# microsoft/gated-graph-neural-network-samples

Measured on AMD Instinct MI355X. Metric: node-state updates/sec on QM9-shaped graphs, h=100, 4 edge types, higher is better.
Workload: dtype f32

## Files before the change

gated-graph-neural-network-samples_amd/csrc/ggnn_gru_fused.hip:

```cpp
#include "ggnn_split.hpp"
#include "ggnn_gru_cells.hpp"
#include <type_traits>

#ifndef GGNN_COOP_DEPTH
#define GGNN_COOP_DEPTH 1
#endif
#ifndef GGNN_GRU_STAMPS
#define GGNN_GRU_STAMPS 0
#endif
#if GGNN_GRU_STAMPS
#define GGNN_TDBG(a) (a).tdbg
#else
#define GGNN_TDBG(a) ((unsigned long long*)nullptr)
#endif

#ifndef GGNN_GRU_ABLATE
#define GGNN_GRU_ABLATE 0
#endif
#if GGNN_GRU_ABLATE
#define GGNN_ABL(BIT) ((ablate & (BIT)) != 0)
#define GGNN_ABL_PARAM , int ablate
#define GGNN_ABL_ARG , gru_ablate_bits()
static int gru_ablate_bits() { static const int v = [] { const char* e = getenv("GGNN_GRU_DBG"); return e ? atoi(e) : 0; }(); return v; }
#else
// ... 19 lines not shown
                  ImgCfg<32, true>::IMG >= ImgCfg<32, true, kSplitF16x2>::IMG, "bf16x3 images are the larger ones");
    switch (D) {
        case 100: return 3 * (nx + 1) * (sp ? ImgCfg<100, true>::IMG : ImgCfg<100, false>::IMG);
        case 64: return 3 * (nx + 1) * (sp ? ImgCfg<64, true>::IMG : ImgCfg<64, false>::IMG);
        case 32: return 3 * (nx + 1) * (sp ? ImgCfg<32, true>::IMG : ImgCfg<32, false>::IMG);
        default: return 0;
    }
}
#endif

template <int D, bool SPLIT, int FMT = kSplitBf16x3>
__global__ void gru_pack_weights_kernel(const float* __restrict__ Wg, const float* __restrict__ Wc, int nx,
                                        float* __restrict__ out) {
    const int ci = blockIdx.y;
    float* img = out + (size_t)ci * ImgCfg<D, SPLIT, FMT>::IMG;
    if constexpr (SPLIT) gru_fwd_image_pack_split<D, FMT>(Wg, Wc, nx, ci, img, blockIdx.x * blockDim.x + threadIdx.x, gridDim.x * blockDim.x);
    else gru_fwd_image_pack<D>(Wg, Wc, nx, ci, img, blockIdx.x * blockDim.x + threadIdx.x, gridDim.x * blockDim.x);
}

template <int NX>
__host__ __device__ constexpr int gru_stage_image(int pos) {
    return (pos % 3) < 2 ? 2 * (pos / 3) + (pos % 3) : 2 * (NX + 1) + pos / 3;
}

template <int FMT>
__device__ __forceinline__ f32x4 sigmoid4_acc(f32x4 z, f32x4 b_scaled) {
    constexpr float k = -kLog2e * SplitFmt<FMT>::acc_scale;
    return rcp_4(exp2_4(z * k + b_scaled) + 1.0f);
}
template <int FMT>
__device__ __forceinline__ f32x4 tanh4_acc(f32x4 z, f32x4 b_scaled) {
    constexpr float k = 2.0f * kLog2e * SplitFmt<FMT>::acc_scale;
    return 1.0f - 2.0f * rcp_4(exp2_4(z * k + b_scaled) + 1.0f);
}

template <int D>
__device__ __forceinline__ void frag_zero(Frag<D>& f) {
#pragma unroll
    for (int c = 0; c < StageCfg<D>::NC; ++c) f.v[c] = f32x4{0.f, 0.f, 0.f, 0.f};
#pragma unroll
    for (int q = 0; q < StageCfg<D>::NR; ++q) f.r[q] = 0.f;
}

template <int D>
__device__ __forceinline__ void frag_add(Frag<D>& f, const Frag<D>& t) {
#pragma unroll
    for (int c = 0; c < StageCfg<D>::NC; ++c) f.v[c] += t.v[c];
#pragma unroll
    for (int q = 0; q < StageCfg<D>::NR; ++q) f.r[q] += t.r[q];
}

template <int D, int NX, int NW, bool SAVE, bool GATHER, bool SPLIT, bool SAVEX = SAVE, int FORM = 0, int FMT = kSplitBf16x3,
          int TK = kTkRuntime, bool G4AVG = false>
__global__ __launch_bounds__(NW * 64, FORM == 1 ? 2 : 1) void ggnn_gru_fused_kernel(GruFusedArgs a, const float* __restrict__ packed GGNN_ABL_PARAM) {
    static_assert(SPLIT || FMT == kSplitBf16x3, "the f32-MFMA kernels have no operand format");
    using C = StageCfg<D>;
    using I = ImgCfg<D, SPLIT, FMT>;
    using SC = SplitCfg<D, FMT>;
    constexpr bool HALF = FORM != 0;
    constexpr bool DEEP = FORM == 2;
    constexpr int NSLOT = DEEP ? 3 : 2;
    static_assert(!HALF || SPLIT, "the half-stage forms are split-form kernels");
    static_assert(FORM != 1 || NW == 4, "form 1 is the four-wave kernel");
    static_assert(!G4AVG || GATHER, "G4AVG fixes the gather's parameters");
    auto dyn_tk = [&]() -> bool {
        if constexpr (TK == kTkRuntime) return a.tickets != nullptr;
// ... 52 lines not shown
    };
    auto publish = [&]() { if constexpr (SPLIT) dma_wait(); __syncthreads(); };
    auto dma_ha = [&](const float* src, float* dst) { dma_kib_asm<SC::HA_BYTES / 1024, NW>(src, dst, wave, lane); };
    auto dma_hb = [&](const float* src, float* dst) { dma_kib_asm<SC::HB_BYTES / 1024, NW>(src, dst, wave, lane); };
    constexpr int KA = SC::HA_BYTES / 1024, KB = SC::HB_BYTES / 1024;
    const int own_a = KA / NW + (wave < KA % NW ? 1 : 0), own_b = KB / NW + (wave < KB % NW ? 1 : 0);
    auto publish_deep = [&](int own) {
        switch (own) {
            case 0: asm volatile("s_waitcnt vmcnt(0) lgkmcnt(0)" ::: "memory"); break;
            case 1: asm volatile("s_waitcnt vmcnt(1) lgkmcnt(0)" ::: "memory"); break;
            case 2: asm volatile("s_waitcnt vmcnt(2) lgkmcnt(0)" ::: "memory"); break;
            case 3: asm volatile("s_waitcnt vmcnt(3) lgkmcnt(0)" ::: "memory"); break;
            case 4: asm volatile("s_waitcnt vmcnt(4) lgkmcnt(0)" ::: "memory"); break;
            case 5: asm volatile("s_waitcnt vmcnt(5) lgkmcnt(0)" ::: "memory"); break;
            case 6: asm volatile("s_waitcnt vmcnt(6) lgkmcnt(0)" ::: "memory"); break;
            case 7: asm volatile("s_waitcnt vmcnt(7) lgkmcnt(0)" ::: "memory"); break;
            case 8: asm volatile("s_waitcnt vmcnt(8) lgkmcnt(0)" ::: "memory"); break;
            case 9: asm volatile("s_waitcnt vmcnt(9) lgkmcnt(0)" ::: "memory"); break;
            default: asm volatile("s_waitcnt vmcnt(10) lgkmcnt(0)" ::: "memory"); break;
        }
        __builtin_amdgcn_s_barrier();
    };
    static_assert(!DEEP || (SC::HA_BYTES / 1024 + NW - 1) / NW <= 10, "publish_deep covers <= 10 pieces per wave");
    if constexpr (DEEP) {
        dma_ha(packed, ring);
        dma_hb(packed + SC::HA, ring + SLOT);
    } else if constexpr (HALF) dma_ha(packed, ring);
    else dma(packed, ring);

    constexpr int GSEG = NX - 1, GBUF = GSEG & 1;
    constexpr int KI = 4;
    constexpr int G_U = NX == 1 ? NSTAGE : 3 * (NX - 1);
    constexpr bool G_NEXT = (NX == 1);
    int g_beg = 0, g_end = 0;
    int g_i[KI] = {0, 0, 0, 0};
    f32x4 g_n = {0.f, 0.f, 0.f, 0.f};
    float g_den = 1.f, g_rcp = 1.f;
    Frag<D> gt;

    auto g_ptrs = [&](int r, bool on) {
        const int b = ldi_b(a.g_row_ptr, (unsigned)r * 4u), e = ldi_b(a.g_row_ptr, (unsigned)r * 4u + 4u);
        g_beg = on ? b : 0; g_end = on ? e : 0;
        if constexpr (G4AVG) {
            g_n = ld4_b(a.g_nin, (unsigned)r * 16u);
        } else if (a.g_use_avg) {
            if (a.g_T == 4) {
                g_n = ld4_b(a.g_nin, (unsigned)r * 16u);
            } else {
                float deg = 0.f;
                for (int t = 0; t < a.g_T; ++t) deg += a.g_nin[(size_t)r * a.g_T + t];
                g_n = f32x4{deg, 0.f, 0.f, 0.f};
            }
        }
    };
    auto touch = [](auto v) { asm volatile("" :: "v"(v)); };
    auto g_index = [&](int part) {
        if (part != 2) {
            touch(g_beg); touch(g_end);
            g_den = (((g_n.x + g_n.y) + g_n.z) + g_n.w) + 1e-7f;
            if constexpr (NX == 1) g_rcp = 1.0f / g_den;
        }
        if (part != 1) {
#pragma unroll
            for (int j = 0; j < KI; ++j) {
                g_i[j] = 0;
                if (g_beg + j < g_end) g_i[j] = ldi_b(a.g_idx, (unsigned)(g_beg + j) * 4u);
            }
        }
    };
    auto g_rows0 = [&](Frag<D>& f, int part) {
        if (part != 2) { touch(g_i[0]); touch(g_i[1]); touch(g_i[2]); touch(g_i[3]); }
        if (part != 1) {
            load_frag<D>(f, a.g_H, g_i[0], kq);
            load_frag<D>(gt, a.g_H, g_i[1], kq);
        }
    };
    auto g_rows = [&](Frag<D>& f, int k, int part) {
        if (part != 2) { if (g_beg + k - 1 < g_end) frag_add<D>(f, gt); }
        if (part != 1) load_frag<D>(gt, a.g_H, g_i[k], kq);
    };
    auto g_finish = [&](Frag<D>& f) {
        if (g_beg + KI - 1 < g_end) frag_add<D>(f, gt);
        for (int e = g_beg + KI; e < g_end; ++e) {
            load_frag<D>(gt, a.g_H, a.g_idx[e], kq);
            frag_add<D>(f, gt);
        }
        if (g_beg >= g_end) frag_zero<D>(f);
        if (G4AVG || a.g_use_avg) {
            const float den = g_den, r = g_rcp;
            auto dv = [&](float x) {
                if constexpr (NX == 1) { const float q = x * r; return fmaf(fmaf(-den, q, x), r, q); }
                else return x / den;
            };
#pragma unroll
            for (int c = 0; c < NC; ++c) f.v[c] = f32x4{dv(f.v[c].x), dv(f.v[c].y), dv(f.v[c].z), dv(f.v[c].w)};
#pragma unroll
            for (int q = 0; q < NR; ++q) f.r[q] = dv(f.r[q]);
        }
    };

    auto store_x = [&](const Frag<D>& f, int row_) {
        const unsigned ob = ((unsigned)row_ * (unsigned)D + 4u * (unsigned)kq) * 4u;
#pragma unroll
        for (int c = 0; c < NC; ++c) st4_b(a.save_x, ob + 64u * c, f.v[c]);
#pragma unroll
        for (int q = 0; q < NR; ++q) *reinterpret_cast<float*>(reinterpret_cast<char*>(a.save_x) + ob - 16u * (unsigned)kq + (16u * NC + 4u * q + (unsigned)kq) * 4u) = f.r[q];
    };
    Frag<D> hf, xf[2];
    {
        const int t0 = tile_of(tk);
        const bool on = t0 >= 0;
        const int r0 = (on ? t0 : 0) * 16 + li;
        const int r0c = r0 < a.V ? r0 : a.V - 1;
        if constexpr (GATHER) {
            if constexpr (G_NEXT) {
                g_ptrs(r0c, on);
                if (on) { g_index(0); g_rows0(xf[0], 0); g_rows(xf[0], 2, 0); g_rows(xf[0], 3, 0); g_finish(xf[0]); }
                if constexpr (SAVEX) { if (on && r0 < a.V && a.save_x) store_x(xf[0], r0); }
            } else {
                if constexpr (G_U - 5 < 0) g_ptrs(r0c, on);
                if constexpr (G_U - 4 < 0) g_index(0);
                load_frag<D>(xf[0], a.x[0], r0c, kq);
            }
        } else {
// ... 220 lines not shown
        GGNN_STAGE(0, acc_r, xf[0]) GGNN_STAGE(1, acc_u, xf[0]) GGNN_STAGE(2, acc_c, xf[0])
        if constexpr (NX >= 2) { GGNN_STAGE(3, acc_r, xf[1]) GGNN_STAGE(4, acc_u, xf[1]) GGNN_STAGE(5, acc_c, xf[1]) }
        if constexpr (NX >= 3) { GGNN_STAGE(6, acc_r, xf[0]) GGNN_STAGE(7, acc_u, xf[0]) GGNN_STAGE(8, acc_c, xf[0]) }
        GGNN_STAGE(3 * NX, acc_r, hf)
        GGNN_STAGE(3 * NX + 1, acc_u, hf)

        Frag<D> rh;
        if constexpr (coop) {
            const int col = wave * 16 + 4 * kq;
            if (wave < NT && col < D && !GGNN_ABL(2)) {
                const f32x4 r = sigmoid4_acc<FMT>(acc_r[0], ld4(bias_s + col));
                const f32x4 u = sigmoid4_acc<FMT>(acc_u[0], ld4(bias_s + D + col));
                f32x4 hv;
                if constexpr (COOP_REGS) hv = hv_pre;
                else hv = ld4_b(a.h, ((unsigned)rowc * D + col) * 4u);
                if constexpr (SAVE) {
                    if (row < a.V && a.save_r) {
                        st4_b(a.save_r, ((unsigned)row * D + col) * 4u, r);
                        st4_b(a.save_u, ((unsigned)row * D + col) * 4u, u);
                    }
                }
                acc_u[0] = u; acc_r[0] = hv;
                *reinterpret_cast<f32x4*>(rh_x + li * RHP + col) = r * hv;
            }
            __syncthreads();
#pragma unroll
            for (int c = 0; c < NC; ++c) rh.v[c] = *reinterpret_cast<const f32x4*>(rh_x + li * RHP + 16 * c + 4 * kq);
#pragma unroll
            for (int q = 0; q < NR; ++q) rh.r[q] = rh_x[li * RHP + 16 * NC + 4 * q + kq];
        } else if (active && !GGNN_ABL(2)) {
            stage_tail_reduce<D>(acc_r);
            stage_tail_reduce<D>(acc_u);
            if constexpr (C::TAILPACK) {
                constexpr int SH = 16 * ((D % 16) / 4);
                f32x4 ut;
                ut.x = __shfl(acc_r[NT - 1].x, lane + SH); ut.y = __shfl(acc_r[NT - 1].y, lane + SH);
                ut.z = __shfl(acc_r[NT - 1].z, lane + SH); ut.w = __shfl(acc_r[NT - 1].w, lane + SH);
                acc_u[NT - 1] = ut;
            }
#pragma unroll
            for (int nt = 0; nt < NT; ++nt) {
                const int col = nt * 16 + 4 * kq;
                if (col < D) {
                    const f32x4 r = sigmoid4_acc<FMT>(acc_r[nt], ld4(bias_s + col));
                    const f32x4 u = sigmoid4_acc<FMT>(acc_u[nt], ld4(bias_s + D + col));
                    acc_r[nt] = r; acc_u[nt] = u;
                    if constexpr (!SAVE && SPLIT && GATHER) { touch(u.x); touch(u.y); touch(u.z); touch(u.w); }
                    if constexpr (SAVE) {
                        if (row < a.V && a.save_r) {
                            st4_b(a.save_r, ((unsigned)row * D + col) * 4u, r);
                            st4_b(a.save_u, ((unsigned)row * D + col) * 4u, u);
                        }
                    }
                }
            }
#pragma unroll
            for (int c = 0; c < NC; ++c) rh.v[c] = acc_r[c] * hf.v[c];
#pragma unroll
            for (int q = 0; q < NR; ++q) {
                const float t0 = __shfl(acc_r[NT - 1].x, li + 16 * q), t1 = __shfl(acc_r[NT - 1].y, li + 16 * q);
                const float t2 = __shfl(acc_r[NT - 1].z, li + 16 * q), t3 = __shfl(acc_r[NT - 1].w, li + 16 * q);
                const float rr = kq == 0 ? t0 : (kq == 1 ? t1 : (kq == 2 ? t2 : t3));
                rh.r[q] = rr * hf.r[q];
            }
        }

        if (dyn_tk() && tid == 0) tk_slot[(p + 1) & 1] = nb + tk_fetch;
        GGNN_STAGE(3 * NX + 2, acc_c, rh)
#undef GGNN_STAGE
#undef GGNN_HALF_STAGE
#undef GGNN_COOP_STAGE
        tk = tk_next;
        tk_next = dyn_tk() ? __builtin_amdgcn_readfirstlane(tk_slot[(p + 1) & 1]) : tk_next + nb;

        if constexpr (coop) {
            const int col = wave * 16 + 4 * kq;
            if (wave < NT && col < D && row < a.V && !GGNN_ABL(4)) {
                f32x4 c;
                if (a.act == GGNN_ACT_TANH) {
                    c = tanh4_acc<FMT>(acc_c[0], ld4(bias_s + 2 * D + col));
                } else {
                    c = acc_c[0] * SplitFmt<FMT>::acc_scale + ld4(bias_s + 3 * D + col);
                    c.x = fmaxf(c.x, 0.f); c.y = fmaxf(c.y, 0.f); c.z = fmaxf(c.z, 0.f); c.w = fmaxf(c.w, 0.f);
                }
                const f32x4 u = acc_u[0], hv = acc_r[0];
                st4_b(a.h_out, ((unsigned)row * D + col) * 4u, u * hv + (1.0f - u) * c);
                if constexpr (SAVE) { if (a.save_c) st4_b(a.save_c, ((unsigned)row * D + col) * 4u, c); }
            }
            return;
        }
        f32x4 hrem = {0.f, 0.f, 0.f, 0.f};
        if (active) {
            stage_tail_reduce<D>(acc_c);
            if constexpr (C::TAILPACK3) {
                constexpr int SH2 = 32 * ((D % 16) / 4);
                f32x4 ct;
                ct.x = __shfl(acc_r[NT - 1].x, lane + SH2); ct.y = __shfl(acc_r[NT - 1].y, lane + SH2);
                ct.z = __shfl(acc_r[NT - 1].z, lane + SH2); ct.w = __shfl(acc_r[NT - 1].w, lane + SH2);
                acc_c[NT - 1] = ct + acc_c[NT - 1];
            }
#pragma unroll
            for (int q = 0; q < NR; ++q) {
                const float h0 = __shfl(hf.r[q], li), h1 = __shfl(hf.r[q], li + 16);
                const float h2 = __shfl(hf.r[q], li + 32), h3 = __shfl(hf.r[q], li + 48);
                if (kq == q) hrem = f32x4{h0, h1, h2, h3};
            }
        }
        if (active && row < a.V && !GGNN_ABL(4)) {
#pragma unroll
            for (int nt = 0; nt < NT; ++nt) {
                const int col = nt * 16 + 4 * kq;
                if (col < D) {
                    f32x4 hv;
                    if (nt < NC) hv = hf.v[nt];
                    else hv = hrem;
                    f32x4 c;
                    if (a.act == GGNN_ACT_TANH) {
                        c = tanh4_acc<FMT>(acc_c[nt], ld4(bias_s + 2 * D + col));
                    } else {
                        c = acc_c[nt] * SplitFmt<FMT>::acc_scale + ld4(bias_s + 3 * D + col);
                        c.x = fmaxf(c.x, 0.f); c.y = fmaxf(c.y, 0.f); c.z = fmaxf(c.z, 0.f); c.w = fmaxf(c.w, 0.f);
                    }
                    const f32x4 u = acc_u[nt];
                    st4_b(a.h_out, ((unsigned)row * D + col) * 4u, u * hv + (1.0f - u) * c);
                    if constexpr (SAVE) { if (a.save_c) st4_b(a.save_c, ((unsigned)row * D + col) * 4u, c); }
                }
            }
        }
    };
    int p = 0;
    for (; tk < n_main; ++p) run_pass(std::false_type{}, p);
    if constexpr (!HALF) { for (; tk < n_tk; ++p) run_pass(std::true_type{}, p); }
    if (GGNN_TDBG(a) && tid == 0) {
        a.tdbg[4096 + blockIdx.x * 4 + 2] = __builtin_amdgcn_s_memtime();
        a.tdbg[4096 + blockIdx.x * 4 + 3] = __builtin_amdgcn_s_memrealtime();
    }
}

// ... 235 lines not shown
```

gated-graph-neural-network-samples_amd/csrc/ggnn_msg_compact.hip:

```cpp
#include "ggnn_split.hpp"
#include <cstring>
#include <rocprim/device/device_scan.hpp>

namespace ggnn {

#ifndef GGNN_K1C_STAMPS
#define GGNN_K1C_STAMPS 0
#endif

constexpr int kMaxTypesC = 64;
struct TypeRows {
    int row_off[kMaxTypesC + 1]; int tile_off[kMaxTypesC + 1]; int T; int num_nodes;
#if GGNN_K1C_STAMPS
    unsigned long long* tdbg;
#endif
};

static inline size_t align256c(size_t x) { return (x + 255) / 256 * 256; }

__global__ void compact_flags_kernel(const int* __restrict__ src_row_ptr, int V, int T, int* flags) {
    const long long p = (long long)blockIdx.x * blockDim.x + threadIdx.x;
    if (p >= (long long)V * T) return;
    const int t = (int)(p / V), v = (int)(p - (long long)t * V);
    const int s = v * T + t;
    flags[p] = src_row_ptr[s + 1] > src_row_ptr[s] ? 1 : 0;
}

__global__ void compact_fill_kernel(const int* __restrict__ flags, const int* __restrict__ scan, int V, int T,
                                    int* pair_node, int* pair_id, int* type_row_off) {
    const long long p = (long long)blockIdx.x * blockDim.x + threadIdx.x;
    const long long n = (long long)V * T;
    if (p >= n) return;
    const int t = (int)(p / V), v = (int)(p - (long long)t * V);
    const int f = flags[p], c = scan[p];
    pair_id[v * T + t] = f ? c : -1;
    if (f) pair_node[c] = v;
    if (v == 0) type_row_off[t] = c;
    if (p == n - 1) type_row_off[T] = c + f;
}

__global__ void remap_rows_kernel(const int* __restrict__ gather_row, const int* __restrict__ pair_id, int* out, long long M) {
    const long long i = (long long)blockIdx.x * blockDim.x + threadIdx.x;
    if (i < M) out[i] = pair_id[gather_row[i]];
}

static size_t scan_temp_bytes(long long n) {
    size_t bytes = 0;
    (void)rocprim::exclusive_scan(nullptr, bytes, (const int*)nullptr, (int*)nullptr, 0, (size_t)n, rocprim::plus<int>(), (hipStream_t)0);
    return bytes;
}

template <int D, bool SPLIT, int FMT = kSplitBf16x3>
__global__ void edge_weight_pack_kernel(const float* __restrict__ W, float* __restrict__ out) {
    const int t = blockIdx.y;
    float* img = out + (size_t)t * ImgCfg<D, SPLIT, FMT>::IMG;
    const int first = blockIdx.x * blockDim.x + threadIdx.x, stride = gridDim.x * blockDim.x;
    if constexpr (SPLIT) pack_split_image<D, FMT>(StageValue<D>{W + (size_t)t * D * D, 0, 0, D, -1, nullptr, 0, 0, -1}, img, first, stride);
    else pack_stage_image<D>(W + (size_t)t * D * D, 0, 0, D, img, first, stride);
}

template <int D, int NW, bool SPLIT, int FMT = kSplitBf16x3>
__global__ __launch_bounds__(NW * 64, 4)  void msg_transform_compact_kernel(
        const float* __restrict__ h, const int* __restrict__ pair_node, TypeRows tr, const float* __restrict__ packed, float* __restrict__ Hc) {
    using C = StageCfg<D>;
    using I = ImgCfg<D, SPLIT, FMT>;
    constexpr int NT = C::NT;
    extern __shared__ __attribute__((aligned(16))) float img[];
    const int tid = threadIdx.x, lane = tid & 63;
    const int wave = __builtin_amdgcn_readfirstlane(tid >> 6);
    const int li = lane & 15, kq = lane >> 4;

#if GGNN_K1C_STAMPS
#define K1C_T(K) if (tr.tdbg && lane == 0) tr.tdbg[((size_t)blockIdx.x * NW + wave) * 8 + (K)] = (K) == 0 || (K) == 7 ? __builtin_amdgcn_s_memrealtime() : __builtin_amdgcn_s_memtime();
#else
#define K1C_T(K)
#endif
    K1C_T(0)
    K1C_T(6)
    int t = 0;
    while (t + 1 < tr.T && (int)blockIdx.x >= tr.tile_off[t + 1]) ++t;
    const int row_beg = tr.row_off[t], row_end = tr.row_off[t + 1];
    const int n_wt = (row_end - row_beg + 15) / 16;
    const int stride = (tr.tile_off[t + 1] - tr.tile_off[t]) * NW;
    int idx = ((int)blockIdx.x - tr.tile_off[t]) * NW + wave;

    auto row_of = [&](int i) { const int r = row_beg + i * 16 + li; return r < row_end ? r : row_end - 1; };
    Frag<D> a, an;
    int node_0 = 0, node_n = 0;
    if (idx < n_wt) node_0 = pair_node[row_of(idx)];
    if (idx + stride < n_wt) node_n = pair_node[row_of(idx + stride)];
    if constexpr (SPLIT) dma_image_asm<I::IMG_BYTES, NW>(packed + (size_t)t * I::IMG, img, wave, lane);
    else dma_stage_image<D, NW>(packed + (size_t)t * C::IMG, img, wave, lane);
    if (idx < n_wt) load_frag<D>(a, h, node_0, kq);
    K1C_T(1)
    if constexpr (SPLIT) dma_wait();
    __syncthreads();
    K1C_T(2)
#if GGNN_K1C_STAMPS
    int tcount = 0;
#endif

    while (idx < n_wt) {
        const int idx_n = idx + stride;
        if (idx_n < n_wt) load_frag<D>(an, h, node_n, kq);
        if (idx_n + stride < n_wt) node_n = pair_node[row_of(idx_n + stride)];
        f32x4 acc[NT];
        __builtin_amdgcn_sched_barrier(0);
        if constexpr (SPLIT) {
            SFrag<D> sf;
            split_frag<D, FMT>(sf, a);
            stage_mma_split<D, NT, true, false, FMT>(acc, sf, a, img, li, kq);
// ... 39 lines not shown
    for (int t = 0; t < tr.T; ++t) total_wt += (tr.row_off[t + 1] - tr.row_off[t] + 15) / 16;
    static const int wg_per_cu = [] { const char* e = getenv("GGNN_K1_WG_PER_CU"); return e && atoi(e) == 1 ? 1 : 2; }();
    const long long budget = (long long)wg_per_cu * num_cus();
    long long R = total_wt / (budget * NW);
    if (R < 1) R = 1;
    for (;; ++R) {
        long long blocks = 0;
        for (int t = 0; t < tr.T; ++t) blocks += ((tr.row_off[t + 1] - tr.row_off[t] + 15) / 16 + R * NW - 1) / (R * NW);
        if (blocks <= budget) break;
    }
    tr.tile_off[0] = 0;
    for (int t = 0; t < tr.T; ++t)
        tr.tile_off[t + 1] = tr.tile_off[t] + (int)(((tr.row_off[t + 1] - tr.row_off[t] + 15) / 16 + R * NW - 1) / (R * NW));
    static std::atomic<unsigned long long> lds_ok{0};
    if (C::IMG_BYTES > 48 * 1024) GGNN_CHECK_HIP(allow_dynamic_lds(&msg_transform_compact_kernel<D, NW, SPLIT, FMT>, C::IMG_BYTES, lds_ok));
#if GGNN_K1C_STAMPS
    { const char* e = getenv("GGNN_K1C_TPTR"); tr.tdbg = e ? (unsigned long long*)strtoull(e, nullptr, 10) : nullptr; }
#endif
    hipLaunchKernelGGL((msg_transform_compact_kernel<D, NW, SPLIT, FMT>), dim3(tr.tile_off[tr.T]), dim3(NW * 64), C::IMG_BYTES, st, h, pair_node,
                       tr, (const float*)packed, Hc);
    GGNN_CHECK_HIP(hipGetLastError());
    return GGNN_OK;
}

template <int D>
static int launch_compact(const float* h, const float* W, const int* pair_node, TypeRows& tr, float* packed, float* Hc, int fmt,
                          hipStream_t st) {
    if (SplitCfg<D>::OK && split_matrix_path())
        return gru_launch_fmt(fmt) == kSplitF16x2 ? launch_compact_m<D, true, kSplitF16x2>(h, W, pair_node, tr, packed, Hc, st)
                                                  : launch_compact_m<D, true>(h, W, pair_node, tr, packed, Hc, st);
    return launch_compact_m<D, false>(h, W, pair_node, tr, packed, Hc, st);
}

int gru_panel_supported(int D);
int transform_panel_image_floats(int D);
int transform_panel_dispatch(const float* h, const float* W, const int* pair_node, const int* row_off, int T, int V, int D,
                             float* packed, float* Hc, int fmt, hipStream_t st);

static int stage_img_floats(int D) {
    if (gru_panel_supported(D)) return (D / 64) * transform_panel_image_floats(D);
    const bool sp = split_matrix_path();
    switch (D) {
        case 100: return sp ? ImgCfg<100, true>::IMG : ImgCfg<100, false>::IMG;
        case 64: return sp ? ImgCfg<64, true>::IMG : ImgCfg<64, false>::IMG;
        case 32: return sp ? ImgCfg<32, true>::IMG : ImgCfg<32, false>::IMG;
        default: return 0;
    }
}

}

using namespace ggnn;

extern "C" int ggnn_msg_transform_compact_supported(int D) { return stage_img_floats(D) > 0; }

extern "C" size_t ggnn_compact_workspace_bytes(int V, int T) {
    if (V <= 0 || T <= 0) return 256;
    const size_t n = (size_t)V * T;
    return 2 * align256c(n * sizeof(int)) + align256c(scan_temp_bytes((long long)n)) + 256;
}

extern "C" int ggnn_build_compact_sources(const int32_t* src_row_ptr, int V, int T, int32_t* pair_node, int32_t* pair_id,
                                          int32_t* type_row_off, void* ws, size_t ws_bytes, ggnn_stream_t stream) {
    GGNN_CHECK_ARG(V >= 0 && T > 0 && T <= kMaxTypesC && (long long)V * T < (1LL << 31), "bad sizes V=%d T=%d", V, T);
    GGNN_CHECK_ARG(type_row_off, "null pointer");
    hipStream_t st = (hipStream_t)stream;
// ... 23 lines not shown

extern "C" int ggnn_remap_gather_rows(const int32_t* gather_row, const int32_t* pair_id, int32_t* gather_row_compact, int64_t M,
                                      ggnn_stream_t stream) {
    GGNN_CHECK_ARG(M >= 0, "negative M");
    if (M == 0) return GGNN_OK;
    GGNN_CHECK_ARG(gather_row && pair_id && gather_row_compact, "null pointer");
    hipLaunchKernelGGL(remap_rows_kernel, dim3((unsigned)((M + 255) / 256)), dim3(256), 0, (hipStream_t)stream, gather_row, pair_id,
                       gather_row_compact, (long long)M);
    GGNN_CHECK_HIP(hipGetLastError());
    return GGNN_OK;
}

extern "C" size_t ggnn_msg_transform_compact_workspace_bytes(int D, int T) {
    return (size_t)stage_img_floats(D) * sizeof(float) * (size_t)(T > 0 ? T : 0) + 256;
}

extern "C" int ggnn_edge_weights_pack_f32(const float* W, int T, int D, int fmt, float* packed, ggnn_stream_t stream) {
    GGNN_CHECK_ARG(T > 0 && T <= kMaxTypesC, "bad T=%d", T);
    GGNN_CHECK_ARG(fmt == 0 || fmt == GGNN_GRU_FMT_F16X2 || fmt == GGNN_GRU_FMT_BF16X3, "fmt %d is not a GGNN_GRU_FMT_* value", fmt);
    if (!ggnn_msg_transform_compact_supported(D))
        return fail(GGNN_E_UNSUPPORTED, "no packed edge weights for hidden size %d", D);
    GGNN_CHECK_ARG(W && packed && aligned16(packed), "null or misaligned pointer");
    TypeRows tr{};
    tr.T = T;
    hipStream_t st = (hipStream_t)stream;
    if (gru_panel_supported(D)) return transform_panel_dispatch(nullptr, W, nullptr, tr.row_off, T, 0, D, packed, nullptr, fmt, st);
    switch (D) {
        case 100: return launch_compact<100>(nullptr, W, nullptr, tr, packed, nullptr, fmt, st);
        case 64: return launch_compact<64>(nullptr, W, nullptr, tr, packed, nullptr, fmt, st);
        default: return launch_compact<32>(nullptr, W, nullptr, tr, packed, nullptr, fmt, st);
    }
}

extern "C" int ggnn_msg_transform_compact_f32(const float* h, const float* W, const int32_t* pair_node,
                                              const int64_t* type_row_off, float* Hc, void* ws, size_t ws_bytes, int V, int D,
                                              int T, int fmt, ggnn_stream_t stream) {
    GGNN_CHECK_ARG(V >= 0 && D > 0 && D % 4 == 0 && T > 0 && T <= kMaxTypesC, "bad sizes V=%d D=%d T=%d", V, D, T);
    GGNN_CHECK_ARG(fmt == 0 || fmt == GGNN_GRU_FMT_F16X2 || fmt == GGNN_GRU_FMT_BF16X3, "fmt %d is not a GGNN_GRU_FMT_* value", fmt);
    GGNN_CHECK_ARG(type_row_off, "null pointer");
    if (!ggnn_msg_transform_compact_supported(D))
        return fail(GGNN_E_UNSUPPORTED, "compacted message transform supports hidden sizes 32, 64, 100, 128, 192, 256 (got %d)", D);
    TypeRows tr;
    tr.T = T;
    tr.num_nodes = V;
    tr.tile_off[0] = 0;
    GGNN_CHECK_ARG(type_row_off[0] == 0, "type_row_off must start at 0");
    for (int t = 0; t < T; ++t) {
        GGNN_CHECK_ARG(type_row_off[t] <= type_row_off[t + 1] && type_row_off[t + 1] < (1LL << 31), "type_row_off not monotone");
        tr.row_off[t] = (int)type_row_off[t];
        tr.tile_off[t + 1] = tr.tile_off[t] + (int)((type_row_off[t + 1] - type_row_off[t] + 127) / 128);
    }
    tr.row_off[T] = (int)type_row_off[T];
    if (tr.row_off[T] == 0) return GGNN_OK;
    GGNN_CHECK_ARG(h && pair_node && Hc && ws, "null pointer");
    GGNN_CHECK_ARG(aligned16(h) && (!W || aligned16(W)) && aligned16(Hc) && aligned16(ws), "pointers must be 16-byte aligned");
    if (ws_bytes < ggnn_msg_transform_compact_workspace_bytes(D, T))
        return fail(GGNN_E_WORKSPACE, "compact transform workspace too small");
    hipStream_t st = (hipStream_t)stream;
    float* packed = static_cast<float*>(ws);
    if (gru_panel_supported(D)) return transform_panel_dispatch(h, W, pair_node, tr.row_off, T, V, D, packed, Hc, fmt, st);
    switch (D) {
        case 100: return launch_compact<100>(h, W, pair_node, tr, packed, Hc, fmt, st);
        case 64: return launch_compact<64>(h, W, pair_node, tr, packed, Hc, fmt, st);
        default: return launch_compact<32>(h, W, pair_node, tr, packed, Hc, fmt, st);
    }
}
```

gated-graph-neural-network-samples_amd/csrc/ggnn_propagate.hip:

```cpp
#include "ggnn_common.h"
#include <cstring>

static constexpr int kTileCounters = 1024;

extern "C" size_t ggnn_sparse_propagate_workspace_bytes(int V, int D, int T, int64_t compact_rows) {
    if (V < 0 || D <= 0 || T <= 0) return 0;
    const size_t vd = (size_t)V * D * sizeof(float);
    const size_t hrows = compact_rows >= 0 ? (size_t)(compact_rows > 0 ? compact_rows : 1) * D * sizeof(float)
                                           : (size_t)V * T * D * sizeof(float);
    return hrows + 3 * vd + ggnn_gru_workspace_bytes(V, D) + kTileCounters * sizeof(int32_t) + 6 * 256;
}

static inline char* bump(char*& p, size_t bytes) {
    char* r = p;
    p += (bytes + 255) / 256 * 256;
    return r;
}

struct RnnCell {
    const float* const* w;
    const float* const* b;
    const float* const* packed;
    int64_t M;
};

static int propagate(
        const RnnCell* rnn, const float* h0, int V, int D, int T,
        const int32_t* row_ptr, const int32_t* gather_row, const int32_t* pair_node, const int64_t* type_row_off,
        const float* nin, int use_avg,
        int num_layers, const int32_t* layer_timesteps, const int32_t* res_ptr, const int32_t* res_idx,
        const float* const* edge_w, const float* const* edge_packed, const float* const* edge_bias,
        const float* const* Wg, const float* const* bg, const float* const* Wc, const float* const* bc,
        const float* const* gru_packed, const int32_t* gru_fmt, const int32_t* edge_fmt, int act, int fuse_gather,
        float* const* layer_out, void* ws, size_t ws_bytes, const int32_t* slot_pair, const float* const* attn_factors,
        ggnn_stream_t stream) {
    GGNN_CHECK_ARG(V >= 0 && D > 0 && D % 4 == 0 && T > 0, "bad sizes V=%d D=%d T=%d", V, D, T);
    GGNN_CHECK_ARG(num_layers > 0 && layer_timesteps && res_ptr && layer_out, "bad layer description");
    GGNN_CHECK_ARG(edge_w || edge_packed, "edge weights missing");
    if (rnn) GGNN_CHECK_ARG(rnn->b && (rnn->packed || rnn->w) && rnn->M >= 0, "RNN weights missing");
    else GGNN_CHECK_ARG(bg && bc && (gru_packed || (Wg && Wc)), "GRU weights missing");
    const bool compact = pair_node != nullptr && type_row_off != nullptr;
    GGNN_CHECK_ARG(!rnn || compact, "the RNN cell runs on the compacted transform only (pair_node, type_row_off)");
    if (V == 0) return GGNN_OK;
    GGNN_CHECK_ARG(h0 && row_ptr && ws, "null pointer");
    GGNN_CHECK_ARG(!attn_factors || compact, "propagation attention needs the compacted transform (pair_node, type_row_off)");
    const int64_t rows = compact ? type_row_off[T] : -1;
    if (ws_bytes < ggnn_sparse_propagate_workspace_bytes(V, D, T, rows))
        return ggnn::fail(GGNN_E_WORKSPACE, "propagate workspace too small: %zu < %zu", ws_bytes,
                          ggnn_sparse_propagate_workspace_bytes(V, D, T, rows));
    const size_t vd = (size_t)V * D * sizeof(float);
    char* p = reinterpret_cast<char*>((reinterpret_cast<size_t>(ws) + 255) / 256 * 256);
    float* H = reinterpret_cast<float*>(bump(p, compact ? (size_t)(rows > 0 ? rows : 1) * D * sizeof(float)
                                                       : (size_t)V * T * D * sizeof(float)));
    float* incoming = reinterpret_cast<float*>(bump(p, vd));
    float* ping[2] = {reinterpret_cast<float*>(bump(p, vd)), nullptr};
    ping[1] = reinterpret_cast<float*>(bump(p, vd));
    int32_t* counters = reinterpret_cast<int32_t*>(bump(p, kTileCounters * sizeof(int32_t)));
    void* gru_ws = p;
    const size_t gru_ws_bytes = ggnn_gru_workspace_bytes(V, D);
    int step_no = 0;
    {
        int total_steps = 0;
        for (int l = 0; l < num_layers; ++l) total_steps += layer_timesteps[l] > 0 ? layer_timesteps[l] : 0;
        if (total_steps > kTileCounters) total_steps = kTileCounters;
        if (total_steps > 0) GGNN_CHECK_HIP(hipMemsetAsync(counters, 0, (size_t)total_steps * sizeof(int32_t), (hipStream_t)stream));
    }

    const float* states[64];
    GGNN_CHECK_ARG(num_layers < 63, "too many layers");
    states[0] = h0;
    for (int l = 0; l < num_layers; ++l) {
        const int nres = res_ptr[l + 1] - res_ptr[l];
        GGNN_CHECK_ARG(nres >= 0 && nres <= 6, "layer %d has %d residual inputs (max 6)", l, nres);
        const float* xs[7];
        for (int i = 0; i < nres; ++i) {
            const int src = res_idx[res_ptr[l] + i];
            GGNN_CHECK_ARG(src >= 0 && src <= l, "layer %d: residual index %d refers to a later layer", l, src);
            xs[i] = states[src];
        }
        xs[nres] = incoming;
        const int nx = nres + 1;
        GGNN_CHECK_ARG(layer_out[l], "layer_out[%d] is null", l);
        const float* cur = states[l];
        const int steps = layer_timesteps[l];
        const float* bias_l = edge_bias ? edge_bias[l] : nullptr;
        const bool packed_gru = !rnn && gru_packed && gru_packed[l] && ggnn_gru_is_fused(D) && nx <= 3;
        const int fmt_l = gru_fmt ? gru_fmt[l] : GGNN_GRU_FMT_BF16X3;
        const float* factors_l = attn_factors ? attn_factors[l] : nullptr;
        GGNN_CHECK_ARG(!attn_factors || factors_l, "attn_factors[%d] is null", l);
        const bool gather_in_gru = !rnn && !attn_factors && fuse_gather > 0 && nx <= fuse_gather && packed_gru && ggnn_gru_is_fused(D) == 1 && bias_l == nullptr &&
                                   (unsigned long long)V * T * D < (1ULL << 30);
        const bool panel_rnn = rnn && ggnn_rnn_panel_supported(D, nx);
        const bool gather_in_rnn = rnn && fuse_gather > 0 && nx <= fuse_gather && rnn->packed && rnn->packed[l] &&
                                   (panel_rnn || ggnn_rnn_fused_supported(D, nx)) && bias_l == nullptr &&
                                   (unsigned long long)V * D < (1ULL << 30) && (unsigned long long)(rows > 0 ? rows : 1) * D < (1ULL << 30);
        if (rnn) GGNN_CHECK_ARG(rnn->b[l] && (gather_in_rnn || (rnn->w && rnn->w[l])), "layer %d needs raw RNN weights (no fused cell for it)", l);
        for (int s = 0; s < steps; ++s) {
            int rc;
            if (compact) {
                const bool packed = edge_packed && edge_packed[l];
                rc = ggnn_msg_transform_compact_f32(cur, packed ? nullptr : edge_w[l], pair_node, type_row_off, H,
                                                    packed ? const_cast<float*>(edge_packed[l]) : gru_ws,
                                                    packed ? ggnn_msg_transform_compact_workspace_bytes(D, T) : gru_ws_bytes,
                                                    V, D, T, (packed && edge_fmt) ? edge_fmt[l] : GGNN_GRU_FMT_BF16X3, stream);
            } else {
                GGNN_CHECK_ARG(edge_w && edge_w[l], "dense transform needs raw edge weights");
                rc = ggnn_msg_transform_f32(cur, D, edge_w[l], H, V, D, T, stream);
            }
            if (rc) return rc;
            float* out = (s + 1 == steps) ? layer_out[l] : ping[s & 1];
            static const bool dyn_tiles = [] { const char* e = getenv("GGNN_DYN_TILES"); return !e || atoi(e) != 0; }();
            int32_t* counter = (dyn_tiles && step_no < kTileCounters) ? counters + step_no : nullptr;
            ++step_no;
            if (gather_in_rnn && panel_rnn) {
                rc = ggnn_rnn_panel_gather_f32(xs, nx, cur, rnn->packed[l], rnn->b[l], out, H, rows > 0 ? rows : 1, row_ptr, gather_row,
                                               rnn->M, nin, T, use_avg, nullptr, V, D, act, stream);
            } else if (gather_in_rnn) {
                rc = ggnn_rnn_packed_gather_f32(xs, nx, cur, rnn->packed[l], rnn->b[l], out, H, rows > 0 ? rows : 1, row_ptr, gather_row,
                                                rnn->M, nin, T, use_avg, nullptr, V, D, act, stream);
            } else if (rnn) {
                rc = ggnn_gather_segment_sum_f32(H, row_ptr, gather_row, nin, bias_l, use_avg, incoming, V, D, T, stream);
                if (rc) return rc;
                rc = ggnn_rnn_f32(xs, nx, cur, rnn->w[l], rnn->b[l], out, V, D, act, stream);
            } else if (gather_in_gru) {
                rc = ggnn_gru_packed_gather_f32(xs, nx, cur, gru_packed[l], bg[l], bc[l], out, H, row_ptr, gather_row, nin, T,
                                                use_avg, V, D, act, fmt_l, counter, stream);
            } else {
                rc = factors_l ? ggnn_gather_segment_sum_attn_compact_f32(H, cur, row_ptr, slot_pair, gather_row, factors_l, nin, bias_l,
                                                                          use_avg, incoming, V, D, T, stream)
                               : ggnn_gather_segment_sum_f32(H, row_ptr, gather_row, nin, bias_l, use_avg, incoming, V, D, T, stream);
                if (rc) return rc;
                if (packed_gru)
                    rc = ggnn_gru_packed_f32(xs, nx, cur, gru_packed[l], bg[l], bc[l], out, nullptr, nullptr, nullptr, V, D, act,
                                             fmt_l, counter, stream);
                else {
                    GGNN_CHECK_ARG(Wg && Wc && Wg[l] && Wc[l], "layer %d needs raw GRU weights (no packed images for it)", l);
                    rc = ggnn_gru_f32(xs, nx, cur, Wg[l], bg[l], Wc[l], bc[l], out, gru_ws, gru_ws_bytes, nullptr, nullptr,
                                      nullptr, V, D, act, stream);
                }
            }
            if (rc) return rc;
            cur = out;
        }
        if (steps == 0) {
            GGNN_CHECK_HIP(hipMemcpyAsync(layer_out[l], cur, vd, hipMemcpyDeviceToDevice, (hipStream_t)stream));
        }
// ... 53 lines not shown
```

Measured before the change: 1.296 billion.

## Use permlane swaps for tail packing, reciprocal averaging, and in-transform counter zeroing

Replaces several __shfl-based cross-lane moves in the fused GRU tail with permlane16/32 swap intrinsics. The tail sigmoid is computed once before the rows move, so the packed update values are no longer recomputed. The gather average now uses reciprocal-plus-correction division for more configurations. The per-step dynamic tile counter is reset inside the compact transform kernel, or by a memset on the panel path, instead of in a separate up-front zeroing pass. Together these aim to cut cross-lane traffic, division cost and launch or memset overhead, at the cost of more complex counter-reset ordering.

New measurement: 1.317 billion (median of 6 runs). 1.6% higher.

```diff
diff --git a/gated-graph-neural-network-samples_amd/csrc/ggnn_gru_fused.hip b/gated-graph-neural-network-samples_amd/csrc/ggnn_gru_fused.hip
--- a/gated-graph-neural-network-samples_amd/csrc/ggnn_gru_fused.hip
+++ b/gated-graph-neural-network-samples_amd/csrc/ggnn_gru_fused.hip
@@ -75,6 +75,30 @@
 __device__ __forceinline__ f32x4 tanh4_acc(f32x4 z, f32x4 b_scaled) {
     constexpr float k = 2.0f * kLog2e * SplitFmt<FMT>::acc_scale;
     return 1.0f - 2.0f * rcp_4(exp2_4(z * k + b_scaled) + 1.0f);
+}
+
+__device__ __forceinline__ float row_up16(float x) {
+    const unsigned u = __float_as_uint(x);
+    return __uint_as_float(__builtin_amdgcn_permlane16_swap(u, u, false, false)[1]);
+}
+__device__ __forceinline__ float row_up32(float x) {
+    const unsigned u = __float_as_uint(x);
+    return __uint_as_float(__builtin_amdgcn_permlane32_swap(u, u, false, false)[1]);
+}
+template <int SH>
+__device__ __forceinline__ f32x4 rows_up(f32x4 v) {
+    static_assert(SH == 16 || SH == 32, "whole rows, one or two up");
+    if constexpr (SH == 16) return f32x4{row_up16(v.x), row_up16(v.y), row_up16(v.z), row_up16(v.w)};
+    else return f32x4{row_up32(v.x), row_up32(v.y), row_up32(v.z), row_up32(v.w)};
+}
+__device__ __forceinline__ float row0_elems_to_rows(f32x4 v) {
+    const unsigned a = __builtin_amdgcn_permlane16_swap(__float_as_uint(v.x), __float_as_uint(v.y), false, false)[0];
+    const unsigned b = __builtin_amdgcn_permlane16_swap(__float_as_uint(v.z), __float_as_uint(v.w), false, false)[0];
+    return __uint_as_float(__builtin_amdgcn_permlane32_swap(a, b, false, false)[0]);
+}
+__device__ __forceinline__ f32x4 rows_to_row0_elems(float x) {
+    const float x1 = row_up16(x);
+    return f32x4{x, x1, row_up32(x), row_up32(x1)};
 }
 
 template <int D>
@@ -193,6 +217,7 @@
     constexpr int KI = 4;
     constexpr int G_U = NX == 1 ? NSTAGE : 3 * (NX - 1);
     constexpr bool G_NEXT = (NX == 1);
+    constexpr bool G_RCP = NX == 1 || (FORM != 0 && D != 32);
     int g_beg = 0, g_end = 0;
     int g_i[KI] = {0, 0, 0, 0};
     f32x4 g_n = {0.f, 0.f, 0.f, 0.f};
@@ -219,7 +244,7 @@
         if (part != 2) {
             touch(g_beg); touch(g_end);
             g_den = (((g_n.x + g_n.y) + g_n.z) + g_n.w) + 1e-7f;
-            if constexpr (NX == 1) g_rcp = 1.0f / g_den;
+            if constexpr (G_RCP) g_rcp = 1.0f / g_den;
         }
         if (part != 1) {
 #pragma unroll
@@ -250,7 +275,7 @@
         if (G4AVG || a.g_use_avg) {
             const float den = g_den, r = g_rcp;
             auto dv = [&](float x) {
-                if constexpr (NX == 1) { const float q = x * r; return fmaf(fmaf(-den, q, x), r, q); }
+                if constexpr (G_RCP) { const float q = x * r; return fmaf(fmaf(-den, q, x), r, q); }
                 else return x / den;
             };
 #pragma unroll
@@ -537,18 +562,20 @@
             stage_tail_reduce<D>(acc_r);
             stage_tail_reduce<D>(acc_u);
             if constexpr (C::TAILPACK) {
-                constexpr int SH = 16 * ((D % 16) / 4);
-                f32x4 ut;
-                ut.x = __shfl(acc_r[NT - 1].x, lane + SH); ut.y = __shfl(acc_r[NT - 1].y, lane + SH);
-                ut.z = __shfl(acc_r[NT - 1].z, lane + SH); ut.w = __shfl(acc_r[NT - 1].w, lane + SH);
-                acc_u[NT - 1] = ut;
+                constexpr int KQ = (D % 16) / 4;
+                const f32x4 b = ld4(bias_s + 16 * NC + 4 * kq + (kq < KQ ? 0 : D - 4 * KQ));
+                if (kq < 2 * KQ) acc_r[NT - 1] = sigmoid4_acc<FMT>(acc_r[NT - 1], b);
+                acc_u[NT - 1] = rows_up<16 * KQ>(acc_r[NT - 1]);
             }
 #pragma unroll
             for (int nt = 0; nt < NT; ++nt) {
                 const int col = nt * 16 + 4 * kq;
                 if (col < D) {
-                    const f32x4 r = sigmoid4_acc<FMT>(acc_r[nt], ld4(bias_s + col));
-                    const f32x4 u = sigmoid4_acc<FMT>(acc_u[nt], ld4(bias_s + D + col));
+                    f32x4 r = acc_r[nt], u = acc_u[nt];
+                    if (!(C::TAILPACK && nt == NT - 1)) {
+                        r = sigmoid4_acc<FMT>(acc_r[nt], ld4(bias_s + col));
+                        u = sigmoid4_acc<FMT>(acc_u[nt], ld4(bias_s + D + col));
+                    }
                     acc_r[nt] = r; acc_u[nt] = u;
                     if constexpr (!SAVE && SPLIT && GATHER) { touch(u.x); touch(u.y); touch(u.z); touch(u.w); }
                     if constexpr (SAVE) {
@@ -563,9 +590,14 @@
             for (int c = 0; c < NC; ++c) rh.v[c] = acc_r[c] * hf.v[c];
 #pragma unroll
             for (int q = 0; q < NR; ++q) {
-                const float t0 = __shfl(acc_r[NT - 1].x, li + 16 * q), t1 = __shfl(acc_r[NT - 1].y, li + 16 * q);
-                const float t2 = __shfl(acc_r[NT - 1].z, li + 16 * q), t3 = __shfl(acc_r[NT - 1].w, li + 16 * q);
-                const float rr = kq == 0 ? t0 : (kq == 1 ? t1 : (kq == 2 ? t2 : t3));
+                float rr;
+                if constexpr (NR == 1) {
+                    rr = row0_elems_to_rows(acc_r[NT - 1]);
+                } else {
+                    const float t0 = __shfl(acc_r[NT - 1].x, li + 16 * q), t1 = __shfl(acc_r[NT - 1].y, li + 16 * q);
+                    const float t2 = __shfl(acc_r[NT - 1].z, li + 16 * q), t3 = __shfl(acc_r[NT - 1].w, li + 16 * q);
+                    rr = kq == 0 ? t0 : (kq == 1 ? t1 : (kq == 2 ? t2 : t3));
+                }
                 rh.r[q] = rr * hf.r[q];
             }
         }
@@ -599,16 +631,17 @@
             stage_tail_reduce<D>(acc_c);
             if constexpr (C::TAILPACK3) {
                 constexpr int SH2 = 32 * ((D % 16) / 4);
-                f32x4 ct;
-                ct.x = __shfl(acc_r[NT - 1].x, lane + SH2); ct.y = __shfl(acc_r[NT - 1].y, lane + SH2);
-                ct.z = __shfl(acc_r[NT - 1].z, lane + SH2); ct.w = __shfl(acc_r[NT - 1].w, lane + SH2);
-                acc_c[NT - 1] = ct + acc_c[NT - 1];
-            }
-#pragma unroll
-            for (int q = 0; q < NR; ++q) {
-                const float h0 = __shfl(hf.r[q], li), h1 = __shfl(hf.r[q], li + 16);
-                const float h2 = __shfl(hf.r[q], li + 32), h3 = __shfl(hf.r[q], li + 48);
-                if (kq == q) hrem = f32x4{h0, h1, h2, h3};
+                acc_c[NT - 1] = rows_up<SH2>(acc_r[NT - 1]) + acc_c[NT - 1];
+            }
+            if constexpr (NR == 1) {
+                hrem = rows_to_row0_elems(hf.r[0]);
+            } else {
+#pragma unroll
+                for (int q = 0; q < NR; ++q) {
+                    const float h0 = __shfl(hf.r[q], li), h1 = __shfl(hf.r[q], li + 16);
+                    const float h2 = __shfl(hf.r[q], li + 32), h3 = __shfl(hf.r[q], li + 48);
+                    if (kq == q) hrem = f32x4{h0, h1, h2, h3};
+                }
             }
         }
         if (active && row < a.V && !GGNN_ABL(4)) {
diff --git a/gated-graph-neural-network-samples_amd/csrc/ggnn_msg_compact.hip b/gated-graph-neural-network-samples_amd/csrc/ggnn_msg_compact.hip
--- a/gated-graph-neural-network-samples_amd/csrc/ggnn_msg_compact.hip
+++ b/gated-graph-neural-network-samples_amd/csrc/ggnn_msg_compact.hip
@@ -11,6 +11,7 @@
 constexpr int kMaxTypesC = 64;
 struct TypeRows {
     int row_off[kMaxTypesC + 1]; int tile_off[kMaxTypesC + 1]; int T; int num_nodes;
+    int* zero;
 #if GGNN_K1C_STAMPS
     unsigned long long* tdbg;
 #endif
@@ -77,6 +78,7 @@
 #endif
     K1C_T(0)
     K1C_T(6)
+    if (tr.zero && blockIdx.x == 0 && tid == 0) *tr.zero = 0;
     int t = 0;
     while (t + 1 < tr.T && (int)blockIdx.x >= tr.tile_off[t + 1]) ++t;
     const int row_beg = tr.row_off[t], row_end = tr.row_off[t + 1];
@@ -182,6 +184,8 @@
     return launch_compact_m<D, false>(h, W, pair_node, tr, packed, Hc, st);
 }
 
+int msg_transform_compact_zero(const float* h, const float* W, const int32_t* pair_node, const int64_t* type_row_off, float* Hc,
+                               void* ws, size_t ws_bytes, int V, int D, int T, int fmt, int32_t* zero, ggnn_stream_t stream);
 int gru_panel_supported(int D);
 int transform_panel_image_floats(int D);
 int transform_panel_dispatch(const float* h, const float* W, const int* pair_node, const int* row_off, int T, int V, int D,
@@ -271,17 +275,17 @@
     }
 }
 
-extern "C" int ggnn_msg_transform_compact_f32(const float* h, const float* W, const int32_t* pair_node,
-                                              const int64_t* type_row_off, float* Hc, void* ws, size_t ws_bytes, int V, int D,
-                                              int T, int fmt, ggnn_stream_t stream) {
+int ggnn::msg_transform_compact_zero(const float* h, const float* W, const int32_t* pair_node, const int64_t* type_row_off, float* Hc,
+                                     void* ws, size_t ws_bytes, int V, int D, int T, int fmt, int32_t* zero, ggnn_stream_t stream) {
     GGNN_CHECK_ARG(V >= 0 && D > 0 && D % 4 == 0 && T > 0 && T <= kMaxTypesC, "bad sizes V=%d D=%d T=%d", V, D, T);
     GGNN_CHECK_ARG(fmt == 0 || fmt == GGNN_GRU_FMT_F16X2 || fmt == GGNN_GRU_FMT_BF16X3, "fmt %d is not a GGNN_GRU_FMT_* value", fmt);
     GGNN_CHECK_ARG(type_row_off, "null pointer");
     if (!ggnn_msg_transform_compact_supported(D))
         return fail(GGNN_E_UNSUPPORTED, "compacted message transform supports hidden sizes 32, 64, 100, 128, 192, 256 (got %d)", D);
-    TypeRows tr;
+    TypeRows tr{};
     tr.T = T;
     tr.num_nodes = V;
+    tr.zero = zero;
     tr.tile_off[0] = 0;
     GGNN_CHECK_ARG(type_row_off[0] == 0, "type_row_off must start at 0");
     for (int t = 0; t < T; ++t) {
@@ -290,12 +294,13 @@
         tr.tile_off[t + 1] = tr.tile_off[t] + (int)((type_row_off[t + 1] - type_row_off[t] + 127) / 128);
     }
     tr.row_off[T] = (int)type_row_off[T];
+    hipStream_t st = (hipStream_t)stream;
+    if (zero && (tr.row_off[T] == 0 || gru_panel_supported(D))) GGNN_CHECK_HIP(hipMemsetAsync(zero, 0, sizeof(int32_t), st));
     if (tr.row_off[T] == 0) return GGNN_OK;
     GGNN_CHECK_ARG(h && pair_node && Hc && ws, "null pointer");
     GGNN_CHECK_ARG(aligned16(h) && (!W || aligned16(W)) && aligned16(Hc) && aligned16(ws), "pointers must be 16-byte aligned");
     if (ws_bytes < ggnn_msg_transform_compact_workspace_bytes(D, T))
         return fail(GGNN_E_WORKSPACE, "compact transform workspace too small");
-    hipStream_t st = (hipStream_t)stream;
     float* packed = static_cast<float*>(ws);
     if (gru_panel_supported(D)) return transform_panel_dispatch(h, W, pair_node, tr.row_off, T, V, D, packed, Hc, fmt, st);
     switch (D) {
@@ -304,3 +309,9 @@
         default: return launch_compact<32>(h, W, pair_node, tr, packed, Hc, fmt, st);
     }
 }
+
+extern "C" int ggnn_msg_transform_compact_f32(const float* h, const float* W, const int32_t* pair_node,
+                                              const int64_t* type_row_off, float* Hc, void* ws, size_t ws_bytes, int V, int D,
+                                              int T, int fmt, ggnn_stream_t stream) {
+    return msg_transform_compact_zero(h, W, pair_node, type_row_off, Hc, ws, ws_bytes, V, D, T, fmt, nullptr, stream);
+}
diff --git a/gated-graph-neural-network-samples_amd/csrc/ggnn_propagate.hip b/gated-graph-neural-network-samples_amd/csrc/ggnn_propagate.hip
--- a/gated-graph-neural-network-samples_amd/csrc/ggnn_propagate.hip
+++ b/gated-graph-neural-network-samples_amd/csrc/ggnn_propagate.hip
@@ -1,5 +1,10 @@
 #include "ggnn_common.h"
 #include <cstring>
+
+namespace ggnn {
+int msg_transform_compact_zero(const float* h, const float* W, const int32_t* pair_node, const int64_t* type_row_off, float* Hc,
+                               void* ws, size_t ws_bytes, int V, int D, int T, int fmt, int32_t* zero, ggnn_stream_t stream);
+}
 
 static constexpr int kTileCounters = 1024;
 
@@ -59,7 +64,8 @@
     void* gru_ws = p;
     const size_t gru_ws_bytes = ggnn_gru_workspace_bytes(V, D);
     int step_no = 0;
-    {
+    const bool zero_in_transform = compact && rows > 0 && ggnn_gru_is_fused(D) == 1;
+    if (!zero_in_transform) {
         int total_steps = 0;
         for (int l = 0; l < num_layers; ++l) total_steps += layer_timesteps[l] > 0 ? layer_timesteps[l] : 0;
         if (total_steps > kTileCounters) total_steps = kTileCounters;
@@ -97,21 +103,22 @@
         if (rnn) GGNN_CHECK_ARG(rnn->b[l] && (gather_in_rnn || (rnn->w && rnn->w[l])), "layer %d needs raw RNN weights (no fused cell for it)", l);
         for (int s = 0; s < steps; ++s) {
             int rc;
+            static const bool dyn_tiles = [] { const char* e = getenv("GGNN_DYN_TILES"); return !e || atoi(e) != 0; }();
+            int32_t* counter = (dyn_tiles && step_no < kTileCounters) ? counters + step_no : nullptr;
+            ++step_no;
             if (compact) {
                 const bool packed = edge_packed && edge_packed[l];
-                rc = ggnn_msg_transform_compact_f32(cur, packed ? nullptr : edge_w[l], pair_node, type_row_off, H,
-                                                    packed ? const_cast<float*>(edge_packed[l]) : gru_ws,
-                                                    packed ? ggnn_msg_transform_compact_workspace_bytes(D, T) : gru_ws_bytes,
-                                                    V, D, T, (packed && edge_fmt) ? edge_fmt[l] : GGNN_GRU_FMT_BF16X3, stream);
+                rc = ggnn::msg_transform_compact_zero(cur, packed ? nullptr : edge_w[l], pair_node, type_row_off, H,
+                                                      packed ? const_cast<float*>(edge_packed[l]) : gru_ws,
+                                                      packed ? ggnn_msg_transform_compact_workspace_bytes(D, T) : gru_ws_bytes,
+                                                      V, D, T, (packed && edge_fmt) ? edge_fmt[l] : GGNN_GRU_FMT_BF16X3,
+                                                      zero_in_transform ? counter : nullptr, stream);
             } else {
                 GGNN_CHECK_ARG(edge_w && edge_w[l], "dense transform needs raw edge weights");
                 rc = ggnn_msg_transform_f32(cur, D, edge_w[l], H, V, D, T, stream);
             }
             if (rc) return rc;
             float* out = (s + 1 == steps) ? layer_out[l] : ping[s & 1];
-            static const bool dyn_tiles = [] { const char* e = getenv("GGNN_DYN_TILES"); return !e || atoi(e) != 0; }();
-            int32_t* counter = (dyn_tiles && step_no < kTileCounters) ? counters + step_no : nullptr;
-            ++step_no;
             if (gather_in_rnn && panel_rnn) {
                 rc = ggnn_rnn_panel_gather_f32(xs, nx, cur, rnn->packed[l], rnn->b[l], out, H, rows > 0 ? rows : 1, row_ptr, gather_row,
                                                rnn->M, nin, T, use_avg, nullptr, V, D, act, stream);
```
